# ath92/splat-renderer

Hardware: AMD Instinct MI355X
Metric: Msplats/sec (higher is better)
Workload: dtype f32

## Files before the change

include/splat.h:

```cpp
#ifndef SPLAT_H
#define SPLAT_H

#include <stddef.h>
#include <stdint.h>

#ifdef __cplusplus
extern "C" {
#endif

#define SPLAT_ABI_VERSION 3

#define SPLAT_OK 0
#define SPLAT_ERR_INVALID (-1)
#define SPLAT_ERR_HIP (-2)
#define SPLAT_ERR_OOM (-3)
#define SPLAT_ERR_CAPACITY (-4)
#define SPLAT_ERR_STATE (-5)
#define SPLAT_ERR_NO_DEVICE (-6)
#define SPLAT_ERR_COMM (-7)
#define SPLAT_ERR_RETRY (-8)

typedef struct splat_ctx splat_ctx;
typedef struct splat_sorter splat_sorter;
typedef struct splat_binner splat_binner;
typedef struct splat_comm splat_comm;

#define SPLAT_PROPS_BYTES 32
#define SPLAT_PROJECTED_BYTES 32
#define SPLAT_SORT_BLOCK 3840

enum {
    SPLAT_STAGE_PROJECT = 0,
    SPLAT_STAGE_SORT = 1,
    SPLAT_STAGE_BIN = 2,
    SPLAT_STAGE_COMPOSITE = 3,
    SPLAT_STAGE_EXCHANGE = 4,
    SPLAT_STAGE_BIN_SCATTER = 5,
    SPLAT_STAGE_BIN_PASS2 = 6,
    SPLAT_STAGE_BIN_TILE_SORT = 7,
    SPLAT_STAGE_COUNT = 8
};

int splat_ctx_create(int device_ordinal, splat_ctx **out);
int splat_ctx_create_on_stream(int device_ordinal, void *hip_stream, splat_ctx **out);
void splat_ctx_destroy(splat_ctx *ctx);
const char *splat_last_error(splat_ctx *ctx);
int splat_sync(splat_ctx *ctx);
int splat_abi_version(void);
int splat_set_timing(splat_ctx *ctx, int enabled);
#define SPLAT_TIMING_COUNT_ENTRIES 0x80000000u
int splat_set_timing_stages(splat_ctx *ctx, uint32_t stage_mask);
int splat_set_timing_sampling(splat_ctx *ctx, uint32_t every);
int splat_stage_time_ms(splat_ctx *ctx, int stage, float *ms);
int splat_stage_time_stats(splat_ctx *ctx, int stage, uint32_t *samples, double *total_ms);
int splat_timing_consumed(splat_ctx *ctx, uint64_t *staged, uint64_t *consumed);

int splat_buf_alloc(splat_ctx *ctx, size_t bytes, void **dptr);
int splat_buf_free(splat_ctx *ctx, void *dptr);
int splat_buf_upload(splat_ctx *ctx, void *dst_dptr, const void *src_host, size_t bytes);
int splat_buf_download(splat_ctx *ctx, void *dst_host, const void *src_dptr, size_t bytes);
int splat_buf_zero(splat_ctx *ctx, void *dptr, size_t bytes);
int splat_buf_copy(splat_ctx *ctx, void *dst_dptr, const void *src_dptr, size_t bytes);

int splat_update_props(splat_ctx *ctx, const void *positions, const void *curvature, uint32_t n,
                       void *props);
int splat_update_props_planes(splat_ctx *ctx, const void *positions, const void *curvature, uint32_t n,
                              void *pos_radius, void *color_opacity);
int splat_props_to_planes(splat_ctx *ctx, const void *props, uint32_t n, void *pos_radius, void *color_opacity);

int splat_project(splat_ctx *ctx, const float *uniforms, const void *pos_radius,
                  uint32_t pr_stride_vec4, uint32_t n, void *projected, void *keys, void *payload,
                  uint32_t n_padded);

int splat_extract_keys(splat_ctx *ctx, const void *projected, uint32_t n, uint32_t n_padded,
                       void *keys, void *payload);

int splat_sort_create(splat_ctx *ctx, uint32_t capacity, splat_sorter **out);
void splat_sort_destroy(splat_sorter *s);
uint32_t splat_sort_capacity(const splat_sorter *s);
void *splat_sort_keys(splat_sorter *s);
void *splat_sort_payload(splat_sorter *s);
int splat_sort_run(splat_sorter *s, uint32_t n, uint32_t bit_begin, uint32_t bit_end);
void *splat_sort_sorted_payload(splat_sorter *s);
void *splat_sort_sorted_keys(splat_sorter *s);
int splat_probe_lds_atomic_order(splat_ctx *ctx, uint64_t *mismatches);
int splat_sort_set_mode(splat_sorter *s, int mode);
int splat_rank_status(splat_ctx *ctx, int *policy, int *atomics_ordered, uint32_t *order_faults);
#ifdef SPLAT_TEST_HOOKS
int splat_debug_inject_order_fault(splat_ctx *ctx, uint32_t tile, uint32_t position);
int splat_debug_set_tile_order(splat_ctx *ctx, const void *order_dptr);
int splat_debug_set_tile_sort_order(splat_ctx *ctx, const void *order_dptr);
int splat_debug_rerun_tile_sort(splat_ctx *ctx, splat_binner *binner);
int splat_debug_tile_sort_launches(splat_ctx *ctx, uint32_t *launches);
int splat_debug_lds_rate(splat_ctx *ctx, int kind, uint32_t workgroups_per_cu, uint32_t iters, float *ms);
#endif
int splat_composite_forget_history(splat_ctx *ctx);
int splat_composite_options(splat_ctx *ctx, int kernel, int ahead, int predict);

int splat_scan_u32(splat_ctx *ctx, const void *in, void *out, uint32_t n, void *total_dptr);

int splat_bin_create(splat_ctx *ctx, uint32_t tile_size, splat_binner **out);
void splat_bin_destroy(splat_binner *b);
int splat_bin_run(splat_binner *b, const void *projected, uint32_t n_splats, const void *sorted,
                  uint32_t n_sorted, uint32_t width, uint32_t height, uint32_t tile_row0,
                  uint32_t tile_row1);
uint32_t splat_bin_tile_size(const splat_binner *b);
int splat_bin_counts(splat_binner *b, void **dptr);
int splat_bin_offsets(splat_binner *b, void **dptr);
int splat_bin_indices(splat_binner *b, void **dptr);
int splat_bin_total(splat_binner *b, uint64_t *total_pairs);
#define SPLAT_FRAME_ORDER_DEFAULT (-1)
#define SPLAT_FRAME_SORT_FIRST 0
#define SPLAT_FRAME_TILE_FIRST 1
int splat_bin_set_frame_order(splat_binner *b, int order);
int splat_bin_dims(splat_binner *b, uint32_t *ntx, uint32_t *nty);

int splat_validate_tile_order(splat_ctx *ctx, const void *projected, const void *tile_offsets,
                              uint32_t num_tiles, const void *tile_indices, uint64_t total_pairs,
                              uint64_t *violations_host);

#define SPLAT_COMPOSITE_FRONT_TO_BACK 0
#define SPLAT_COMPOSITE_REFERENCE_LITERAL 1
#define SPLAT_RECORDS_PROJECTED 0
#define SPLAT_RECORDS_COMPACT 1
#define SPLAT_RECORDS_DISC48 2
#define SPLAT_RECORDS_LIT32 3
#define SPLAT_FOOTPRINT_ISOTROPIC 0
#define SPLAT_FOOTPRINT_DISC 1
#define SPLAT_FOOTPRINT_ELLIPSOID 2
#define SPLAT_FOOTPRINT_SURFEL 3
typedef struct splat_composite_cfg {
    uint32_t mode;
    uint32_t early_out;
    uint32_t tile_size;
    uint32_t tile_row0;
    uint32_t tile_row1;
    uint32_t record_format;
    uint32_t prelit;
    uint32_t footprint;
} splat_composite_cfg;
int splat_lit_colors(splat_ctx *ctx, const void *color_opacity, uint32_t color_stride_vec4,
                     const void *normals, uint32_t normal_stride_vec4, uint32_t n, void *lit);
int splat_composite(splat_ctx *ctx, const splat_composite_cfg *cfg, const void *color_opacity,
                    uint32_t color_stride_vec4, const void *normals, uint32_t normal_stride_vec4,
                    const void *projected, const void *tile_indices, const void *tile_counts,
                    const void *tile_offsets, uint32_t width, uint32_t height, void *out_rgba8,
                    void *out_rgba32f, void *consumed_dptr);

typedef struct splat_aov {
    void *depth_f32;
    void *alpha_f32;
    void *id_u32;
} splat_aov;
int splat_composite_aov(splat_ctx *ctx, const splat_composite_cfg *cfg, const void *color_opacity,
                        uint32_t color_stride_vec4, const void *normals, uint32_t normal_stride_vec4,
                        const void *projected, const void *tile_indices, const void *tile_counts,
                        const void *tile_offsets, uint32_t width, uint32_t height, void *out_rgba8,
                        void *out_rgba32f, void *consumed_dptr, const splat_aov *aov);
int splat_composite_aov_depth(splat_ctx *ctx, const splat_composite_cfg *cfg, const void *color_opacity,
                              uint32_t color_stride_vec4, const void *normals, uint32_t normal_stride_vec4,
                              const void *projected, const void *tile_indices, const void *tile_counts,
                              const void *tile_offsets, uint32_t width, uint32_t height, void *out_rgba8,
                              void *out_rgba32f, void *consumed_dptr, const splat_aov *aov, const void *depth_f32,
                              uint32_t depth_stride_floats);

int splat_render_frame(splat_ctx *ctx, splat_sorter *sorter, splat_binner *binner,
                       const splat_composite_cfg *cfg, const float *uniforms, const void *props,
                       const void *normals, uint32_t n, uint32_t width, uint32_t height,
                       void *projected, void *out_rgba8, void *out_rgba32f);
int splat_render_frame_planes(splat_ctx *ctx, splat_sorter *sorter, splat_binner *binner,
                              const splat_composite_cfg *cfg, const float *uniforms,
                              const void *pos_radius, const void *color_opacity, const void *normals,
                              uint32_t n, uint32_t width, uint32_t height, void *projected,
                              void *out_rgba8, void *out_rgba32f);
int splat_render_frame_aov(splat_ctx *ctx, splat_sorter *sorter, splat_binner *binner,
                           const splat_composite_cfg *cfg, const float *uniforms, const void *props,
// ... 257 lines not shown
```

splat_renderer_amd/_lib.py:

```python
import ctypes as C
import os

_HERE = os.path.dirname(os.path.abspath(__file__))
LIB_PATH = os.environ.get("SPLAT_LIB_PATH") or os.path.join(_HERE, "libsplat_hip.so")

OK = 0
ERR_NAMES = {-1: "INVALID", -2: "HIP", -3: "OOM", -4: "CAPACITY", -5: "STATE", -6: "NO_DEVICE", -7: "COMM", -8: "RETRY"}
ERR_CAPACITY, ERR_RETRY = -4, -8
RENDER_AGAIN = (ERR_CAPACITY, ERR_RETRY)

STAGE_PROJECT, STAGE_SORT, STAGE_BIN, STAGE_COMPOSITE, STAGE_EXCHANGE, STAGE_BIN_SCATTER, STAGE_BIN_PASS2, STAGE_BIN_TILE_SORT = range(8)
STAGE_NAMES = ("project", "sort", "bin", "composite", "exchange", "bin_scatter", "bin_second_pass", "bin_tile_sort")
TIMING_COUNT_ENTRIES = 0x80000000
MODE_FRONT_TO_BACK, MODE_REFERENCE_LITERAL = 0, 1
RECORDS_PROJECTED, RECORDS_COMPACT, RECORDS_DISC48, RECORDS_LIT32 = 0, 1, 2, 3
FOOTPRINT_ISOTROPIC, FOOTPRINT_DISC, FOOTPRINT_ELLIPSOID, FOOTPRINT_SURFEL = 0, 1, 2, 3
U32_MAX = 0xFFFFFFFF
DEPTH_DISTANCE, DEPTH_Z = 0, 1


class SplatError(RuntimeError):
    def __init__(self, code, msg):
        super().__init__(f"libsplat_hip error {ERR_NAMES.get(code, code)}: {msg}")
        self.code = code
# ... 117 lines not shown
    "splat_tsdf_mesh_emit": (_i, [_vp, C.POINTER(TsdfGrid), _vp, _vp, _vp, C.c_uint64, _vp, _vp, _vp]),
    "splat_adam_step": (_i, [_vp, _vp, _vp, _vp, _vp, _u32, _u32, _u32, _f64, _f64, _f64, _f64, _f64, _f64, _vp]),
    "splat_density_accumulate": (_i, [_vp, _vp, _vp, _u32, _u32, _u32, _vp, _vp, _vp, _vp]),
    "splat_density_accumulate_abs": (_i, [_vp, _vp, _vp, _u32, _u32, _u32, _vp, _vp, _vp, _vp]),
    "splat_densify_plan_workspace_bytes": (C.c_uint64, [_u32]),
    "splat_densify_plan": (_i, [_vp, _vp, _vp, _vp, _vp, _vp, _u32, C.POINTER(DensifyCfg), _vp, C.c_uint64, _vp, C.POINTER(_u32),
                                C.POINTER(_u32)]),
    "splat_densify_geometry": (_i, [_vp, _vp, _u32, _vp, _vp, _vp, C.POINTER(DensifyCfg), _vp, _vp]),
    "splat_densify_rows": (_i, [_vp, _vp, _u32, _vp, _vp, _u32, _u32]),
    "splat_mcmc_sample_workspace_bytes": (C.c_uint64, [_u32]),
    "splat_mcmc_sample": (_i, [_vp, _vp, _u32, _u32, _u32, _f64, C.c_uint64, _vp, C.c_uint64, _vp, _vp, _vp, C.POINTER(_u32)]),
    "splat_mcmc_apply": (_i, [_vp, _vp, _vp, _vp, _u32, _u32, _u32, _f64, C.POINTER(McmcPlanes)]),
    "splat_mcmc_noise": (_i, [_vp, _vp, _vp, _vp, _vp, _u32, _f64, _u32, C.c_uint64]),
    "splat_knn_workspace_bytes": (C.c_uint64, [_u32]),
    "splat_knn_mean_sq": (_i, [_vp, _vp, _vp, _u32, _u32, _vp, C.c_uint64, _vp, _vp]),
    "splat_extract_keys":(_i, [_vp, _vp, _u32, _u32, _vp, _vp]),
    "splat_sort_create": (_i, [_vp, _u32, _pvp]),
    "splat_sort_destroy": (None, [_vp]),
    "splat_sort_capacity": (_u32, [_vp]),
    "splat_sort_keys": (_vp, [_vp]),
    "splat_sort_payload": (_vp, [_vp]),
    "splat_sort_run": (_i, [_vp, _u32, _u32, _u32]),
    "splat_sort_sorted_payload": (_vp, [_vp]),
    "splat_sort_sorted_keys": (_vp, [_vp]),
    "splat_probe_lds_atomic_order": (_i, [_vp, C.POINTER(C.c_uint64)]),
    "splat_sort_set_mode": (_i, [_vp, _i]),
    "splat_rank_status": (_i, [_vp, C.POINTER(_i), C.POINTER(_i), C.POINTER(_u32)]),
    "splat_composite_forget_history": (_i, [_vp]),
    "splat_composite_options": (_i, [_vp, _i, _i, _i]),
    "splat_scan_u32": (_i, [_vp, _vp, _vp, _u32, _vp]),
    "splat_bin_create": (_i, [_vp, _u32, _pvp]),
    "splat_bin_destroy": (None, [_vp]),
    "splat_bin_run": (_i, [_vp, _vp, _u32, _vp, _u32, _u32, _u32, _u32, _u32]),
    "splat_bin_tile_size": (_u32, [_vp]),
    "splat_bin_counts": (_i, [_vp, _pvp]),
    "splat_bin_offsets": (_i, [_vp, _pvp]),
    "splat_bin_indices": (_i, [_vp, _pvp]),
    "splat_bin_total": (_i, [_vp, C.POINTER(C.c_uint64)]),
    "splat_bin_set_frame_order": (_i, [_vp, _i]),
    "splat_bin_dims": (_i, [_vp, C.POINTER(_u32), C.POINTER(_u32)]),
    "splat_validate_tile_order": (_i, [_vp, _vp, _vp, _u32, _vp, C.c_uint64, C.POINTER(C.c_uint64)]),
    "splat_lit_colors": (_i, [_vp, _vp, _u32, _vp, _u32, _u32, _vp]),
    "splat_composite": (_i, [_vp, C.POINTER(CompositeCfg), _vp, _u32, _vp, _u32, _vp, _vp, _vp, _vp, _u32, _u32,
                             _vp, _vp, _vp]),
    "splat_render_frame": (_i, [_vp, _vp, _vp, C.POINTER(CompositeCfg), C.POINTER(C.c_float), _vp, _vp, _u32, _u32,
                                _u32, _vp, _vp, _vp]),
    "splat_render_frame_planes": (_i, [_vp, _vp, _vp, C.POINTER(CompositeCfg), C.POINTER(C.c_float), _vp, _vp, _vp, _u32,
                                       _u32, _u32, _vp, _vp, _vp]),
    "splat_composite_aov": (_i, [_vp, C.POINTER(CompositeCfg), _vp, _u32, _vp, _u32, _vp, _vp, _vp, _vp, _u32, _u32,
                                 _vp, _vp, _vp, C.POINTER(Aov)]),
    "splat_render_frame_aov": (_i, [_vp, _vp, _vp, C.POINTER(CompositeCfg), C.POINTER(C.c_float), _vp, _vp, _u32, _u32,
                                    _u32, _vp, _vp, _vp, C.POINTER(Aov)]),
    "splat_render_frame_planes_aov": (_i, [_vp, _vp, _vp, C.POINTER(CompositeCfg), C.POINTER(C.c_float), _vp, _vp, _vp,
                                           _u32, _u32, _u32, _vp, _vp, _vp, C.POINTER(Aov)]),
    "splat_project_slice": (_i, [_vp, C.POINTER(C.c_float), _vp, _u32, _u32, _u32, _vp]),
    "splat_project_slice_compact": (_i, [_vp, C.POINTER(C.c_float), _vp, _u32, _u32, _u32, _vp]),
    "splat_project_slice_disc": (_i, [_vp, C.POINTER(C.c_float), _vp, _u32, _vp, _u32, _u32, _u32, _vp]),
    "splat_expand_compact": (_i, [_vp, _vp, _u32, _u32, _vp]),
    "splat_band_frame": (_i, [_vp, _vp, _vp, C.POINTER(CompositeCfg), _vp, _vp, _vp, _u32, _u32, _u32, _vp, _vp, _vp]),
    "splat_band_settle": (_i, [_vp, _vp, _vp, C.POINTER(_u32), C.POINTER(C.c_uint64)]),
    "splat_band_kept": (_i, [_vp, _vp, C.POINTER(_u32)]),
    "splat_band_keys": (_i, [_vp, _vp, _vp, _u32, _u32, _u32, _u32, _u32, _u32, C.POINTER(_u32)]),
    "splat_sdf_gradients": (_i, [_vp, _vp, _u32, _vp, _u32, _vp]),
    "splat_sdf_update_positions": (_i, [_vp, _vp, _vp, _u32, _vp]),
    "splat_sdf_scale_factors": (_i, [_vp, _vp, _u32, _vp, _u32, _vp]),
    "splat_sdf_curvature": (_i, [_vp, _vp, _vp, _u32, _vp]),
    "splat_sdf_seed_positions": (_i, [_vp, C.POINTER(C.c_float), C.POINTER(C.c_float), _u32, C.c_uint64, _vp]),
    "splat_sdf_generate": (_i, [_vp, _vp, _u32, C.POINTER(C.c_float), C.POINTER(C.c_float), C.c_uint64, _vp, _u32, _u32, _vp, _vp, _vp, _vp]),
    "splat_point_frame": (_i, [_vp, _vp, C.POINTER(C.c_float), _vp, _u32, _vp, _u32, _vp, _u32, _u32, _u32, _u32, _vp, _vp, _vp, _vp]),
    "splat_comm_unique_id": (_i, [_vp]),
    "splat_comm_init": (_i, [_vp, _i, _i, _vp, _pvp]),
    "splat_comm_destroy": (None, [_vp]),
    "splat_comm_rank": (_i, [_vp, C.POINTER(_i), C.POINTER(_i)]),
    "splat_comm_count": (_i, [_vp, C.POINTER(_i), C.POINTER(_i)]),
    "splat_allgather_records": (_i, [_vp, _vp, _vp, _vp, _sz]),
}
COMM_ID_BYTES = 128
HOOK_SIGNATURES = {
    "splat_debug_inject_order_fault": (_i, [_vp, _u32, _u32]),
    "splat_debug_set_tile_order": (_i, [_vp, _vp]),
    "splat_debug_set_tile_sort_order": (_i, [_vp, _vp]),
    "splat_debug_rerun_tile_sort": (_i, [_vp, _vp]),
    "splat_debug_tile_sort_launches": (_i, [_vp, C.POINTER(_u32)]),
    "splat_debug_lds_rate": (_i, [_vp, _i, _u32, _u32, C.POINTER(C.c_float)]),
}
HOOKS_LIB_PATH = os.path.join(_HERE, "libsplat_hip_hooks.so")

_lib = None


class _Bound:

    def __getattr__(self, name):
        if name in HOOK_SIGNATURES:
            raise AttributeError(f"libsplat_hip: {name} is a test hook: the shipped library does not carry it; run with "
                                 f"SPLAT_LIB_PATH={HOOKS_LIB_PATH} (the -DSPLAT_TEST_HOOKS build)")
        raise AttributeError(f"libsplat_hip: {name} is not declared in splat_renderer_amd._lib.SIGNATURES")


def load():
    global _lib
    if _lib is not None:
        return _lib
    if not os.path.exists(LIB_PATH):
        raise ImportError(
            f"{LIB_PATH} not found: build it with `python -c 'import __graft_entry__ as g; g.build()'` "
            "(hipcc --offload-arch=gfx950). splat_renderer_amd has no CPU fallback.")
    dll = C.CDLL(LIB_PATH)
    lib = _Bound()
    for name, (res, args) in SIGNATURES.items():
        fn = getattr(dll, name)
        fn.restype = res
        fn.argtypes = args
        setattr(lib, name, fn)
    lib.has_hooks = hasattr(dll, "splat_debug_inject_order_fault")
    if lib.has_hooks:
        for name, (res, args) in HOOK_SIGNATURES.items():
            fn = getattr(dll, name)
            fn.restype = res
            fn.argtypes = args
            setattr(lib, name, fn)
    lib._dll = dll
    _lib = lib
    return lib


def check(rc, ctx=None):
    if rc != OK:
        msg = load().splat_last_error(ctx)
        raise SplatError(rc, msg.decode("utf-8", "replace") if msg else "")
    return rc
```

splat_renderer_amd/csrc/tile_sort.hip:

```cpp
#include "common.h"
#include "block_scan.h"
#include "variant.h"

#include <cstdlib>

constexpr uint32_t TS_THREADS = 256, TS_WAVES = 4;
constexpr uint32_t TS_LONG_ITEMS = 24;
constexpr uint32_t TS_LDS_ELEMS = 5888;
constexpr uint32_t TS_CHUNK_ITEMS = 16;

struct TileSortShared {
    uint32_t wave_hist[TS_WAVES][256];
    uint32_t digit_base[256];
    uint32_t wave_sums[TS_WAVES];
    uint32_t kmin, kmax;
};

__device__ __forceinline__ void tile_list_out(uint2 *s_el, uint32_t n, uint32_t *__restrict__ out, uint32_t *frame_flags, bool inject,
                                              uint32_t inject_pos, uint32_t tid) {
    const uint32_t lane = tid & 63, w = tid >> 6;
    if (inject) {
        if (tid == 0 && n >= inject_pos + 2u) {
            const uint2 a = s_el[inject_pos];
            s_el[inject_pos] = s_el[inject_pos + 1];
            s_el[inject_pos + 1] = a;
        }
        __syncthreads();
    }
    bool bad = false;
    for (uint32_t s0 = 0; s0 * 63u < n; s0 += 4 * TS_WAVES) {
        uint2 a[4];
#pragma unroll
        for (uint32_t i = 0; i < 4; ++i) {
            const uint32_t p = (s0 + i * TS_WAVES + w) * 63u + lane;
            a[i] = s_el[p < n ? p : n - 1];
        }
#pragma unroll
        for (uint32_t i = 0; i < 4; ++i) {
            const uint32_t p = (s0 + i * TS_WAVES + w) * 63u + lane;
            if (p < n && lane < 63) out[p] = a[i].y;
            const uint32_t bx = (uint32_t)__builtin_amdgcn_update_dpp(0, (int)a[i].x, 0x130, 0xf, 0xf, false);
            const uint32_t by = (uint32_t)__builtin_amdgcn_update_dpp(0, (int)a[i].y, 0x130, 0xf, 0xf, false);
#ifndef TS_NO_ORDER_CHECK
            const unsigned long long ka = ((unsigned long long)a[i].x << 32) | a[i].y, kb = ((unsigned long long)bx << 32) | by;
            if (p + 1 < n && lane < 63) bad |= ka >= kb;
#endif
        }
    }
    if (__any(bad) && lane == 0) atomicOr(frame_flags, FRAME_FLAG_ORDER);
}

#ifdef SPLAT_TEST_HOOKS
#define TS_HOOK_PARAMS , uint32_t inject_tile, uint32_t inject_pos, const uint32_t *__restrict__ order
#define TS_HOOK_ARGS , inject, inject_pos, ctx->debug_sort_order
#else
#define TS_HOOK_PARAMS
#define TS_HOOK_ARGS
#endif
template <bool RANK_ATOMIC, uint32_t TS_MAX_ITEMS, bool LAST_CLASS>
__global__ __launch_bounds__(TS_THREADS, TS_MAX_ITEMS <= 8 ? 6 : TS_MAX_ITEMS <= 12 ? 5 : TS_MAX_ITEMS <= 16 ? 4 : 3) void k_tile_sort(const uint32_t *__restrict__ offsets, uint32_t tiles,
                                                                                    uint32_t n_above, uint2 *vals, uint2 *scratch,
                                                                                    uint32_t *__restrict__ out_idx,
                                                                                    uint32_t *__restrict__ counts,
                                                                                    uint32_t *__restrict__ frame_flags TS_HOOK_PARAMS) {
    static_assert(TS_MAX_ITEMS % 4 == 0, "items are processed in groups of four");
    constexpr uint32_t TS_CAP = TS_MAX_ITEMS * TS_THREADS < TS_LDS_ELEMS ? TS_MAX_ITEMS * TS_THREADS : TS_LDS_ELEMS;
    __shared__ TileSortShared sh;
    __shared__ uint2 s_el[TS_CAP];
    uint32_t *run_base = reinterpret_cast<uint32_t *>(s_el);
    const uint32_t tid = threadIdx.x, lane = tid & 63, w = tid >> 6;
#ifdef SPLAT_TEST_HOOKS
    const uint32_t t = order ? order[blockIdx.x] : blockIdx.x;
#else
    const uint32_t t = blockIdx.x;
    constexpr uint32_t inject_tile = 0xffffffffu, inject_pos = 0;
#endif
    const uint32_t base = offsets[t], n = offsets[t + 1] - base;
    if (counts && tid == 0) {
        counts[t] = n;
        if (n > TS_MAX_ITEMS * TS_THREADS) atomicAdd(frame_flags + 2, 1u);
    }
    if (n <= n_above || (!LAST_CLASS && n > TS_CAP)) return;
    uint2 *src = vals + base, *dst = scratch + base;
    const bool in_lds = !LAST_CLASS || n <= TS_CAP;

    if (tid == 0) {
        sh.kmin = 0xffffffffu;
        sh.kmax = 0;
    }
    __syncthreads();

    uint32_t lo = 0xffffffffu, hi = 0;
    const uint32_t items = ((n + TS_THREADS - 1) / TS_THREADS + 3u) & ~3u;
    const uint32_t wbase = w * items * 64 + lane;
    uint2 el[TS_MAX_ITEMS];
    if (in_lds) {
#pragma unroll
        for (uint32_t g = 0; g < TS_MAX_ITEMS; g += 4) {
            if (g < items) {
#pragma unroll
                for (uint32_t i = g; i < g + 4; ++i) {
                    const uint32_t p = wbase + i * 64;
                    el[i] = src[p < n ? p : n - 1];
                }
            }
        }
#pragma unroll
        for (uint32_t g = 0; g < TS_MAX_ITEMS; g += 4) {
            if (g < items) {
#pragma unroll
                for (uint32_t i = g; i < g + 4; ++i) {
                    lo = min(lo, el[i].x);
                    hi = max(hi, el[i].x);
                }
            }
        }
    } else {
        for (uint32_t p = tid; p < n; p += TS_THREADS) {
            const uint32_t k = src[p].x;
            lo = min(lo, k);
            hi = max(hi, k);
        }
    }
#pragma unroll
    for (int d = 32; d >= 1; d >>= 1) {
        lo = min(lo, (uint32_t)__shfl_xor((int)lo, d));
        hi = max(hi, (uint32_t)__shfl_xor((int)hi, d));
    }
    if (lane == 0) {
        atomicMin(&sh.kmin, lo);
        atomicMax(&sh.kmax, hi);
    }
    __syncthreads();
    const uint32_t kmin = sh.kmin, range = sh.kmax - kmin;
    const uint32_t passes = range == 0 ? 0u : (32u - (uint32_t)__builtin_clz(range) + 7u) / 8u;

    if (in_lds) {
        if (passes == 0) {
#pragma unroll
            for (uint32_t g = 0; g < TS_MAX_ITEMS; g += 4) {
                if (g < items) {
#pragma unroll
                    for (uint32_t i = g; i < g + 4; ++i)
                        if (wbase + i * 64 < n) s_el[wbase + i * 64] = el[i];
                }
            }
            __syncthreads();
        }
        for (uint32_t pass = 0; pass < passes; ++pass) {
            const uint32_t shift = pass * 8;
            for (uint32_t i = tid; i < TS_WAVES * 256; i += TS_THREADS) (&sh.wave_hist[0][0])[i] = 0;
            __syncthreads();
            uint32_t rank[TS_MAX_ITEMS];
#pragma unroll
            for (uint32_t g = 0; g < TS_MAX_ITEMS; g += 4) {
                if (g < items) {
                    if (pass > 0) {
#pragma unroll
                        for (uint32_t i = g; i < g + 4; ++i) {
                            const uint32_t p = wbase + i * 64;
                            el[i] = s_el[p < n ? p : n - 1];
                        }
                    }
#pragma unroll
                    for (uint32_t i = g; i < g + 4; ++i) {
                        const uint32_t p = wbase + i * 64;
                        rank[i] = 0;
                        if (p < n) rank[i] = wave_rank<RANK_ATOMIC>(sh.wave_hist[w], ((el[i].x - kmin) >> shift) & 255u);
                    }
                }
            }
            __syncthreads();
            const uint32_t c0 = sh.wave_hist[0][tid], c1 = sh.wave_hist[1][tid], c2 = sh.wave_hist[2][tid], c3 = sh.wave_hist[3][tid];
            const uint32_t excl = block_exclusive_scan<true>((c0 + c1) + (c2 + c3), sh.wave_sums);
            sh.wave_hist[0][tid] = excl;
            sh.wave_hist[1][tid] = excl + c0;
            sh.wave_hist[2][tid] = excl + c0 + c1;
            sh.wave_hist[3][tid] = excl + c0 + c1 + c2;
            __syncthreads();
#pragma unroll
            for (uint32_t g = 0; g < TS_MAX_ITEMS; g += 4) {
                if (g < items) {
                    uint32_t pos[4];
#pragma unroll
                    for (uint32_t i = g; i < g + 4; ++i) pos[i - g] = sh.wave_hist[w][((el[i].x - kmin) >> shift) & 255u] + rank[i];
#pragma unroll
                    for (uint32_t i = g; i < g + 4; ++i)
                        if (wbase + i * 64 < n) s_el[pos[i - g]] = el[i];
                }
            }
            __syncthreads();
        }
        tile_list_out(s_el, n, out_idx + base, frame_flags, t == inject_tile, inject_pos, tid);
        return;
    }

    constexpr uint32_t CH_ITEMS = TS_MAX_ITEMS < TS_CHUNK_ITEMS ? TS_MAX_ITEMS : TS_CHUNK_ITEMS;
    for (uint32_t pass = 0; pass < passes; ++pass) {
        const uint32_t shift = pass * 8;
        sh.digit_base[tid] = 0;
        __syncthreads();
        for (uint32_t p = tid; p < n; p += TS_THREADS) atomicAdd(&sh.digit_base[((src[p].x - kmin) >> shift) & 255u], 1u);
        __syncthreads();
        const uint32_t tot = sh.digit_base[tid];
        const uint32_t start = block_exclusive_scan<true>(tot, sh.wave_sums);
        run_base[tid] = start;
        __syncthreads();
        for (uint32_t c0 = 0; c0 < n; c0 += CH_ITEMS * TS_THREADS) {
            for (uint32_t i = tid; i < TS_WAVES * 256; i += TS_THREADS) (&sh.wave_hist[0][0])[i] = 0;
            __syncthreads();
            uint2 el[CH_ITEMS];
            uint32_t rank[CH_ITEMS];
#pragma unroll
            for (uint32_t i = 0; i < CH_ITEMS; ++i) {
                const uint32_t p = c0 + w * (CH_ITEMS * 64) + i * 64 + lane;
                el[i] = src[p < n ? p : n - 1];
                rank[i] = 0;
                if (p < n) rank[i] = wave_rank<RANK_ATOMIC>(sh.wave_hist[w], ((el[i].x - kmin) >> shift) & 255u);
            }
            __syncthreads();
            const uint32_t dcount = ts_wave_prefixes(sh.wave_hist, tid);
            const uint32_t rb = run_base[tid];
            sh.digit_base[tid] = rb;
            run_base[tid] = rb + dcount;
            __syncthreads();
#pragma unroll
            for (uint32_t i = 0; i < CH_ITEMS; ++i) {
                const uint32_t p = c0 + w * (CH_ITEMS * 64) + i * 64 + lane;
                if (p < n) {
                    const uint32_t d = ((el[i].x - kmin) >> shift) & 255u;
                    dst[sh.digit_base[d] + sh.wave_hist[w][d] + rank[i]] = el[i];
                }
            }
            __syncthreads();
        }
        uint2 *tmp = src; src = dst; dst = tmp;
        __threadfence_block();
        __syncthreads();
    }
    bool bad = false;
    for (uint32_t p = tid; p < n; p += TS_THREADS) {
        const bool inj = t == inject_tile && n >= inject_pos + 2u;
        uint2 a = src[p];
        if (inj && (p == inject_pos || p == inject_pos + 1)) a = src[p == inject_pos ? p + 1 : p - 1];
        out_idx[base + p] = a.y;
        if (p + 1 < n) {
            uint2 b = src[p + 1];
            if (inj && (p + 1 == inject_pos || p + 1 == inject_pos + 1)) b = src[p + 1 == inject_pos ? p + 2 : p];
            bad |= a.x > b.x || (a.x == b.x && a.y >= b.y);
        }
    }
    if (__any(bad) && lane == 0) atomicOr(frame_flags, FRAME_FLAG_ORDER);
}

int tile_sort_launch(splat_ctx *ctx, const TileSortArgs &a) {
    uint32_t *const counts = a.counts, *const short_class_io = a.short_class_io;
    {
        int prc = ctx_resolve_rank_mode(ctx);
        if (prc != SPLAT_OK) return prc;
    }
    const bool ra = rank_atomic_ok(ctx, true);
#ifdef SPLAT_TEST_HOOKS
    const uint32_t inject = ctx->inject_order_fault ? ctx->inject_order_fault - 1u : 0xffffffffu;
    const uint32_t inject_pos = ctx->inject_order_position;
    ctx->inject_order_fault = 0;
#endif
    const bool one_class = (a.band_tiles ? a.band_tiles : a.tiles) <= 4200u;
    static const uint32_t force_short = [] {
        const char *e = getenv("SPLAT_TILE_SORT_SHORT");
        const int v = e ? atoi(e) : 0;
        return (v == 8 || v == 12 || v == 16) ? (uint32_t)v : 0u;
    }();
    const uint32_t short_items = force_short ? force_short : a.mean_list < 320u ? 8u : a.mean_list < 1152u ? 12u : 16u;
    const uint32_t short_cap = short_items * TS_THREADS;
    auto launch_class = [&](uint32_t items, bool last, uint32_t above, uint32_t *class_counts) {
        return variant_dispatch(
            [&](auto ra_, auto items_, auto last_) {
                if constexpr (items_.value != (int)TS_LONG_ITEMS || last_.value) {
                    launch_kernel(ctx, NO_STAGE, k_tile_sort<ra_.value, (uint32_t)items_.value, last_.value>, dim3(a.tiles), dim3(TS_THREADS), a.offsets,
                                  a.tiles, above, a.vals, a.scratch, a.out_idx, class_counts, a.frame_flags TS_HOOK_ARGS);
                    return true;
                } else return false;
            },
            ra, OneOf<8, 12, 16, (int)TS_LONG_ITEMS>{(int)items}, last);
    };
    bool ok, no_long = false;
    if (one_class) {
        ok = launch_class(TS_LONG_ITEMS, true, 0u, counts);
    } else {
        no_long = a.long_tiles_hint == 0u && short_class_io && *short_class_io == short_items;
        if (short_class_io) *short_class_io = short_items;
        ok = launch_class(short_items, no_long, 0u, counts);
        if (ok && !no_long) ok = launch_class(TS_LONG_ITEMS, true, short_cap, nullptr);
    }
    if (!ok) return ctx_fail(ctx, SPLAT_ERR_INVALID, "k_tile_sort: no kernel for this class");
#ifdef SPLAT_TEST_HOOKS
    ctx->tile_sort_launches = one_class || no_long ? 1u : 2u;
#endif
    LAUNCH_CHECK(ctx, "k_tile_sort");
    return SPLAT_OK;
}

#ifdef SPLAT_TEST_HOOKS
extern "C" int splat_debug_set_tile_sort_order(splat_ctx *ctx, const void *order_dptr) {
    if (!ctx) return ctx_fail(nullptr, SPLAT_ERR_INVALID, "ctx is NULL");
    ctx->debug_sort_order = (const uint32_t *)order_dptr;
    return SPLAT_OK;
}

extern "C" int splat_debug_tile_sort_launches(splat_ctx *ctx, uint32_t *launches) {
    if (!ctx || !launches) return ctx_fail(nullptr, SPLAT_ERR_INVALID, "ctx/launches is NULL");
    *launches = ctx->tile_sort_launches;
    return SPLAT_OK;
}

extern "C" int splat_debug_inject_order_fault(splat_ctx *ctx, uint32_t tile, uint32_t position) {
    if (!ctx) return ctx_fail(nullptr, SPLAT_ERR_INVALID, "ctx is NULL");
    ARG_CHECK(ctx, tile != 0xffffffffu);
    ARG_CHECK(ctx, position < 0x3fffffffu);
    ctx->inject_order_fault = tile + 1u;
    ctx->inject_order_position = position;
    return SPLAT_OK;
}
#endif
```

splat_renderer_amd/host.py:

```python
import ctypes as C

import numpy as np

from . import _lib
from ._lib import CompositeCfg, SplatError, check

U32_MAX = 0xFFFFFFFF


class Buffer:

    def __init__(self, device, ptr, size, owned=True):
        self.device, self.ptr, self.size, self._owned = device, ptr, int(size), owned
        self._host_shadow = None

    def destroy(self):
        if self._owned and self.ptr:
            check(self.device.lib.splat_buf_free(self.device.ctx, self.ptr), self.device.ctx)
        self.ptr = None

    def write(self, array, offset=0):
        a = np.ascontiguousarray(array)
        if offset + a.nbytes > self.size:
            raise ValueError("write past the end of the buffer")
# ... 19 lines not shown


class _Queue:
    def __init__(self, device):
        self._d = device

    def writeBuffer(self, buffer, offset, data):
        buffer.write(data, offset)

    def submit(self, _command_buffers=None):
        pass

    def onSubmittedWorkDone(self):
        self._d.sync()


class CommandEncoder:

    def finish(self):
        return None


class Device:

    def __init__(self, ordinal=0, stream=None):
        self.lib = _lib.load()
        p = C.c_void_p()
        if stream is None:
            check(self.lib.splat_ctx_create(ordinal, C.byref(p)))
        else:
            check(self.lib.splat_ctx_create_on_stream(ordinal, C.c_void_p(stream), C.byref(p)))
        self.ctx = p
        self.ordinal = ordinal
        self.queue = _Queue(self)
        self.lastProjector = None
        self.lastBinner = None

    def createBuffer(self, size):
        p = C.c_void_p()
        check(self.lib.splat_buf_alloc(self.ctx, int(size), C.byref(p)), self.ctx)
        return Buffer(self, p.value, size)

    def createBufferFrom(self, array):
        a = np.ascontiguousarray(array)
        return self.createBuffer(max(a.nbytes, 16)).write(a)

    def wrap(self, ptr, size):
        return Buffer(self, int(ptr), size, owned=False)

    def createCommandEncoder(self):
        return CommandEncoder()

    def sync(self):
        check(self.lib.splat_sync(self.ctx), self.ctx)

    def setTiming(self, enabled=True):
        check(self.lib.splat_set_timing(self.ctx, int(enabled)), self.ctx)

    def stageTimeMs(self, stage):
        ms = C.c_float()
        check(self.lib.splat_stage_time_ms(self.ctx, stage, C.byref(ms)), self.ctx)
        return float(ms.value)

    def rankStatus(self):
        pol, ordered, faults = C.c_int(), C.c_int(), C.c_uint32()
        check(self.lib.splat_rank_status(self.ctx, C.byref(pol), C.byref(ordered), C.byref(faults)), self.ctx)
        return {"policy": ("checked", "atomic", "ballot")[pol.value], "atomicsOrdered": bool(ordered.value == 1),
                "orderFaults": int(faults.value)}

    def forgetCompositeHistory(self):
        check(self.lib.splat_composite_forget_history(self.ctx), self.ctx)

    def compositeOptions(self, kernel=None, ahead=0, predict=None):
        k = -1 if kernel is None else {"quadrant": 0, "pixel": 1}[kernel]
        check(self.lib.splat_composite_options(self.ctx, k, int(ahead), -1 if predict is None else int(bool(predict))), self.ctx)

    def injectOrderFault(self, tile, position=0):
        check(self.lib.splat_debug_inject_order_fault(self.ctx, int(tile), int(position)), self.ctx)

    def tileSortLaunches(self):
        v = C.c_uint32(0)
        check(self.lib.splat_debug_tile_sort_launches(self.ctx, C.byref(v)), self.ctx)
        return int(v.value)

    def destroy(self):
        if self.ctx:
            self.lib.splat_ctx_destroy(self.ctx)
            self.ctx = None


def _uniform_floats(u):
    if isinstance(u, Buffer):
        if u._host_shadow is None:
            raise SplatError(-1, "uniform buffer was never written")
        u = u._host_shadow.view(np.float32)
    u = np.ascontiguousarray(u, dtype=np.float32)
    return u


class PointManager:

    def __init__(self, device, scene, seed=0, seeding="device"):
        self.device = device
        self.scene, self._seed, self._positions = None, seed, None
        if seeding not in ("device", "host"):
            raise SplatError(-1, f"seeding must be 'device' or 'host', not {seeding!r}")
        self.seeding = seeding
        if hasattr(scene, "getPrimitives"):
            from . import sdf
            if not scene.getPrimitives():
                raise SplatError(-1, "Scene must have at least one primitive")
            self.scene = scene
            self.numPoints = sdf.point_count(scene)
        else:
            if isinstance(scene, (int, np.integer)):
                from .scene import make_scene
                props, _ = make_scene(int(scene))
                scene = np.concatenate([props[:, :3], np.ones((props.shape[0], 1), np.float32)], axis=1)
            self._positions = np.ascontiguousarray(scene, dtype=np.float32)
            self.numPoints = self._positions.shape[0]
        self._buffers = [device.createBuffer(self.numPoints * 16), device.createBuffer(self.numPoints * 16)]
        self._current = 0
        self.reinitialize()

    def reinitialize(self):
        if self.scene is not None:
            from . import sdf
            if self.seeding == "device":
                mn, mx = sdf.seeding_box(self.scene)
                fp = C.POINTER(C.c_float)
                check(self.device.lib.splat_sdf_seed_positions(self.device.ctx, mn.ctypes.data_as(fp), mx.ctypes.data_as(fp), self.numPoints,
                                                               int(self._seed) & 0xFFFFFFFFFFFFFFFF, self._buffers[self._current].ptr),
                      self.device.ctx)
                self._seed += 1
                return
            self._positions = sdf.seed_positions(self.scene, self.numPoints, self._seed)
            self._seed += 1
        self._buffers[self._current].write(self._positions)

    def swap(self):
        self._current = 1 - self._current

    def getCurrentPositionBuffer(self):
        return self._buffers[self._current]

    def getNextPositionBuffer(self):
        return self._buffers[1 - self._current]

    def getNumPoints(self):
        return self.numPoints

    def destroy(self):
        for b in self._buffers:
            b.destroy()


class PropertyPlanes:

    def __init__(self, posRadius, colorOpacity, prelit=False, ownsPosRadius=True):
        self.posRadius, self.colorOpacity, self.prelit, self._owns_pos = posRadius, colorOpacity, prelit, ownsPosRadius

    def destroy(self):
        if self._owns_pos:
            self.posRadius.destroy()
        self.colorOpacity.destroy()

# ... 804 lines not shown
```

Baseline: 15650.

## Alias tile-sort shared state into element LDS and pack ranks to raise occupancy

The tile-sort kernel now overlays its histogram and scan scratch onto the element array in LDS instead of allocating both, and raises the launch-bounds occupancy target for each item class. Ranks are packed two per register in 16-bit halves, keys are pre-offset by kmin, and the per-wave key min/max is gathered through slots instead of LDS atomics. A DPP-based wave scan replaces the generic block scan. The global-memory fallback is split into its own function, and a debug hook reports occupancy. Aliasing forces extra barriers, and the tighter register budget may cause spills.

```diff
diff --git a/include/splat.h b/include/splat.h
--- a/include/splat.h
+++ b/include/splat.h
@@ -92,6 +92,7 @@
 int splat_debug_set_tile_sort_order(splat_ctx *ctx, const void *order_dptr);
 int splat_debug_rerun_tile_sort(splat_ctx *ctx, splat_binner *binner);
 int splat_debug_tile_sort_launches(splat_ctx *ctx, uint32_t *launches);
+int splat_debug_tile_sort_occupancy(splat_ctx *ctx, uint32_t items, int last, int ballot, uint32_t *workgroups_per_cu, uint32_t *lds_cap);
 int splat_debug_lds_rate(splat_ctx *ctx, int kind, uint32_t workgroups_per_cu, uint32_t iters, float *ms);
 #endif
 int splat_composite_forget_history(splat_ctx *ctx);
diff --git a/splat_renderer_amd/_lib.py b/splat_renderer_amd/_lib.py
--- a/splat_renderer_amd/_lib.py
+++ b/splat_renderer_amd/_lib.py
@@ -223,6 +223,7 @@
     "splat_debug_set_tile_sort_order": (_i, [_vp, _vp]),
     "splat_debug_rerun_tile_sort": (_i, [_vp, _vp]),
     "splat_debug_tile_sort_launches": (_i, [_vp, C.POINTER(_u32)]),
+    "splat_debug_tile_sort_occupancy": (_i, [_vp, _u32, _i, _i, C.POINTER(_u32), C.POINTER(_u32)]),
     "splat_debug_lds_rate": (_i, [_vp, _i, _u32, _u32, C.POINTER(C.c_float)]),
 }
 HOOKS_LIB_PATH = os.path.join(_HERE, "libsplat_hip_hooks.so")
diff --git a/splat_renderer_amd/csrc/tile_sort.hip b/splat_renderer_amd/csrc/tile_sort.hip
--- a/splat_renderer_amd/csrc/tile_sort.hip
+++ b/splat_renderer_amd/csrc/tile_sort.hip
@@ -8,13 +8,48 @@
 constexpr uint32_t TS_LONG_ITEMS = 24;
 constexpr uint32_t TS_LDS_ELEMS = 5888;
 constexpr uint32_t TS_CHUNK_ITEMS = 16;
+constexpr uint32_t ts_class_cap(uint32_t items) { return items * TS_THREADS < TS_LDS_ELEMS ? items * TS_THREADS : TS_LDS_ELEMS; }
+constexpr uint32_t ts_class_workgroups(uint32_t items) { return items <= 8 ? 8 : items <= 12 ? 6 : items <= 16 ? 5 : 3; }
 
 struct TileSortShared {
     uint32_t wave_hist[TS_WAVES][256];
     uint32_t digit_base[256];
+    uint32_t run_base[256];
     uint32_t wave_sums[TS_WAVES];
-    uint32_t kmin, kmax;
+    uint32_t kmin_w[TS_WAVES], kmax_w[TS_WAVES];
 };
+static_assert(sizeof(TileSortShared) <= 8 * TS_THREADS * sizeof(uint2), "the view must fit the smallest class's element array (8 per thread, 16 KiB)");
+
+__device__ __forceinline__ uint32_t ts_fresh_v(uint32_t v) {
+    asm volatile("" : "+v"(v));
+    return v;
+}
+__device__ __forceinline__ uint32_t ts_fresh_s(uint32_t v) {
+    asm volatile("" : "+s"(v));
+    return v;
+}
+
+template <int CTRL, int ROW_MASK>
+__device__ __forceinline__ uint32_t ts_dpp_add(uint32_t x) {
+    return x + (uint32_t)__builtin_amdgcn_update_dpp(0, (int)x, CTRL, ROW_MASK, 0xf, false);
+}
+__device__ __forceinline__ uint32_t ts_wave_inclusive_scan(uint32_t x) {
+    x = ts_dpp_add<0x111, 0xf>(x);
+    x = ts_dpp_add<0x112, 0xf>(x);
+    x = ts_dpp_add<0x114, 0xf>(x);
+    x = ts_dpp_add<0x118, 0xf>(x);
+    x = ts_dpp_add<0x142, 0xa>(x);
+    x = ts_dpp_add<0x143, 0xc>(x);
+    return x;
+}
+__device__ __forceinline__ uint32_t ts_block_exclusive_scan(uint32_t v, uint32_t *wave_sums, uint32_t lane, uint32_t w) {
+    const uint32_t incl = ts_wave_inclusive_scan(v);
+    if (lane == 63) wave_sums[w] = incl;
+    __syncthreads();
+    const uint32_t before = waves_before(wave_sums, w);
+    __syncthreads();
+    return before + incl - v;
+}
 
 __device__ __forceinline__ void tile_list_out(uint2 *s_el, uint32_t n, uint32_t *__restrict__ out, uint32_t *frame_flags, bool inject,
                                               uint32_t inject_pos, uint32_t tid) {
@@ -50,152 +85,33 @@
     if (__any(bad) && lane == 0) atomicOr(frame_flags, FRAME_FLAG_ORDER);
 }
 
-#ifdef SPLAT_TEST_HOOKS
-#define TS_HOOK_PARAMS , uint32_t inject_tile, uint32_t inject_pos, const uint32_t *__restrict__ order
-#define TS_HOOK_ARGS , inject, inject_pos, ctx->debug_sort_order
-#else
-#define TS_HOOK_PARAMS
-#define TS_HOOK_ARGS
-#endif
-template <bool RANK_ATOMIC, uint32_t TS_MAX_ITEMS, bool LAST_CLASS>
-__global__ __launch_bounds__(TS_THREADS, TS_MAX_ITEMS <= 8 ? 6 : TS_MAX_ITEMS <= 12 ? 5 : TS_MAX_ITEMS <= 16 ? 4 : 3) void k_tile_sort(const uint32_t *__restrict__ offsets, uint32_t tiles,
-                                                                                    uint32_t n_above, uint2 *vals, uint2 *scratch,
-                                                                                    uint32_t *__restrict__ out_idx,
-                                                                                    uint32_t *__restrict__ counts,
-                                                                                    uint32_t *__restrict__ frame_flags TS_HOOK_PARAMS) {
-    static_assert(TS_MAX_ITEMS % 4 == 0, "items are processed in groups of four");
-    constexpr uint32_t TS_CAP = TS_MAX_ITEMS * TS_THREADS < TS_LDS_ELEMS ? TS_MAX_ITEMS * TS_THREADS : TS_LDS_ELEMS;
-    __shared__ TileSortShared sh;
-    __shared__ uint2 s_el[TS_CAP];
-    uint32_t *run_base = reinterpret_cast<uint32_t *>(s_el);
-    const uint32_t tid = threadIdx.x, lane = tid & 63, w = tid >> 6;
-#ifdef SPLAT_TEST_HOOKS
-    const uint32_t t = order ? order[blockIdx.x] : blockIdx.x;
-#else
-    const uint32_t t = blockIdx.x;
-    constexpr uint32_t inject_tile = 0xffffffffu, inject_pos = 0;
-#endif
-    const uint32_t base = offsets[t], n = offsets[t + 1] - base;
-    if (counts && tid == 0) {
-        counts[t] = n;
-        if (n > TS_MAX_ITEMS * TS_THREADS) atomicAdd(frame_flags + 2, 1u);
-    }
-    if (n <= n_above || (!LAST_CLASS && n > TS_CAP)) return;
-    uint2 *src = vals + base, *dst = scratch + base;
-    const bool in_lds = !LAST_CLASS || n <= TS_CAP;
-
-    if (tid == 0) {
-        sh.kmin = 0xffffffffu;
-        sh.kmax = 0;
-    }
-    __syncthreads();
-
-    uint32_t lo = 0xffffffffu, hi = 0;
-    const uint32_t items = ((n + TS_THREADS - 1) / TS_THREADS + 3u) & ~3u;
-    const uint32_t wbase = w * items * 64 + lane;
-    uint2 el[TS_MAX_ITEMS];
-    if (in_lds) {
-#pragma unroll
-        for (uint32_t g = 0; g < TS_MAX_ITEMS; g += 4) {
-            if (g < items) {
-#pragma unroll
-                for (uint32_t i = g; i < g + 4; ++i) {
-                    const uint32_t p = wbase + i * 64;
-                    el[i] = src[p < n ? p : n - 1];
-                }
-            }
-        }
-#pragma unroll
-        for (uint32_t g = 0; g < TS_MAX_ITEMS; g += 4) {
-            if (g < items) {
-#pragma unroll
-                for (uint32_t i = g; i < g + 4; ++i) {
-                    lo = min(lo, el[i].x);
-                    hi = max(hi, el[i].x);
-                }
-            }
-        }
-    } else {
-        for (uint32_t p = tid; p < n; p += TS_THREADS) {
-            const uint32_t k = src[p].x;
-            lo = min(lo, k);
-            hi = max(hi, k);
-        }
-    }
+__device__ __forceinline__ uint32_t ts_key_range(TileSortShared &sh, uint32_t lo, uint32_t hi, uint32_t lane, uint32_t w, uint32_t &kmin) {
 #pragma unroll
     for (int d = 32; d >= 1; d >>= 1) {
         lo = min(lo, (uint32_t)__shfl_xor((int)lo, d));
         hi = max(hi, (uint32_t)__shfl_xor((int)hi, d));
     }
     if (lane == 0) {
-        atomicMin(&sh.kmin, lo);
-        atomicMax(&sh.kmax, hi);
+        sh.kmin_w[w] = lo;
+        sh.kmax_w[w] = hi;
     }
     __syncthreads();
-    const uint32_t kmin = sh.kmin, range = sh.kmax - kmin;
-    const uint32_t passes = range == 0 ? 0u : (32u - (uint32_t)__builtin_clz(range) + 7u) / 8u;
-
-    if (in_lds) {
-        if (passes == 0) {
-#pragma unroll
-            for (uint32_t g = 0; g < TS_MAX_ITEMS; g += 4) {
-                if (g < items) {
-#pragma unroll
-                    for (uint32_t i = g; i < g + 4; ++i)
-                        if (wbase + i * 64 < n) s_el[wbase + i * 64] = el[i];
-                }
-            }
-            __syncthreads();
-        }
-        for (uint32_t pass = 0; pass < passes; ++pass) {
-            const uint32_t shift = pass * 8;
-            for (uint32_t i = tid; i < TS_WAVES * 256; i += TS_THREADS) (&sh.wave_hist[0][0])[i] = 0;
-            __syncthreads();
-            uint32_t rank[TS_MAX_ITEMS];
-#pragma unroll
-            for (uint32_t g = 0; g < TS_MAX_ITEMS; g += 4) {
-                if (g < items) {
-                    if (pass > 0) {
-#pragma unroll
-                        for (uint32_t i = g; i < g + 4; ++i) {
-                            const uint32_t p = wbase + i * 64;
-                            el[i] = s_el[p < n ? p : n - 1];
-                        }
-                    }
-#pragma unroll
-                    for (uint32_t i = g; i < g + 4; ++i) {
-                        const uint32_t p = wbase + i * 64;
-                        rank[i] = 0;
-                        if (p < n) rank[i] = wave_rank<RANK_ATOMIC>(sh.wave_hist[w], ((el[i].x - kmin) >> shift) & 255u);
-                    }
-                }
-            }
-            __syncthreads();
-            const uint32_t c0 = sh.wave_hist[0][tid], c1 = sh.wave_hist[1][tid], c2 = sh.wave_hist[2][tid], c3 = sh.wave_hist[3][tid];
-            const uint32_t excl = block_exclusive_scan<true>((c0 + c1) + (c2 + c3), sh.wave_sums);
-            sh.wave_hist[0][tid] = excl;
-            sh.wave_hist[1][tid] = excl + c0;
-            sh.wave_hist[2][tid] = excl + c0 + c1;
-            sh.wave_hist[3][tid] = excl + c0 + c1 + c2;
-            __syncthreads();
-#pragma unroll
-            for (uint32_t g = 0; g < TS_MAX_ITEMS; g += 4) {
-                if (g < items) {
-                    uint32_t pos[4];
-#pragma unroll
-                    for (uint32_t i = g; i < g + 4; ++i) pos[i - g] = sh.wave_hist[w][((el[i].x - kmin) >> shift) & 255u] + rank[i];
-#pragma unroll
-                    for (uint32_t i = g; i < g + 4; ++i)
-                        if (wbase + i * 64 < n) s_el[pos[i - g]] = el[i];
-                }
-            }
-            __syncthreads();
-        }
-        tile_list_out(s_el, n, out_idx + base, frame_flags, t == inject_tile, inject_pos, tid);
-        return;
-    }
-
-    constexpr uint32_t CH_ITEMS = TS_MAX_ITEMS < TS_CHUNK_ITEMS ? TS_MAX_ITEMS : TS_CHUNK_ITEMS;
+    kmin = min(min(sh.kmin_w[0], sh.kmin_w[1]), min(sh.kmin_w[2], sh.kmin_w[3]));
+    const uint32_t range = max(max(sh.kmax_w[0], sh.kmax_w[1]), max(sh.kmax_w[2], sh.kmax_w[3])) - kmin;
+    return range == 0 ? 0u : (32u - (uint32_t)__builtin_clz(range) + 7u) / 8u;
+}
+
+template <bool RANK_ATOMIC, uint32_t CH_ITEMS>
+__device__ __forceinline__ void tile_sort_through_global(TileSortShared &sh, uint2 *src, uint2 *dst, uint32_t n, uint32_t *__restrict__ out,
+                                                         uint32_t *frame_flags, bool inject, uint32_t inject_pos, uint32_t tid, uint32_t lane,
+                                                         uint32_t w) {
+    uint32_t lo = 0xffffffffu, hi = 0, kmin;
+    for (uint32_t p = tid; p < n; p += TS_THREADS) {
+        const uint32_t k = src[p].x;
+        lo = min(lo, k);
+        hi = max(hi, k);
+    }
+    const uint32_t passes = ts_key_range(sh, lo, hi, lane, w, kmin);
     for (uint32_t pass = 0; pass < passes; ++pass) {
         const uint32_t shift = pass * 8;
         sh.digit_base[tid] = 0;
@@ -203,8 +119,8 @@
         for (uint32_t p = tid; p < n; p += TS_THREADS) atomicAdd(&sh.digit_base[((src[p].x - kmin) >> shift) & 255u], 1u);
         __syncthreads();
         const uint32_t tot = sh.digit_base[tid];
-        const uint32_t start = block_exclusive_scan<true>(tot, sh.wave_sums);
-        run_base[tid] = start;
+        const uint32_t start = ts_block_exclusive_scan(tot, sh.wave_sums, lane, w);
+        sh.run_base[tid] = start;
         __syncthreads();
         for (uint32_t c0 = 0; c0 < n; c0 += CH_ITEMS * TS_THREADS) {
             for (uint32_t i = tid; i < TS_WAVES * 256; i += TS_THREADS) (&sh.wave_hist[0][0])[i] = 0;
@@ -220,9 +136,9 @@
             }
             __syncthreads();
             const uint32_t dcount = ts_wave_prefixes(sh.wave_hist, tid);
-            const uint32_t rb = run_base[tid];
+            const uint32_t rb = sh.run_base[tid];
             sh.digit_base[tid] = rb;
-            run_base[tid] = rb + dcount;
+            sh.run_base[tid] = rb + dcount;
             __syncthreads();
 #pragma unroll
             for (uint32_t i = 0; i < CH_ITEMS; ++i) {
@@ -240,10 +156,10 @@
     }
     bool bad = false;
     for (uint32_t p = tid; p < n; p += TS_THREADS) {
-        const bool inj = t == inject_tile && n >= inject_pos + 2u;
+        const bool inj = inject && n >= inject_pos + 2u;
         uint2 a = src[p];
         if (inj && (p == inject_pos || p == inject_pos + 1)) a = src[p == inject_pos ? p + 1 : p - 1];
-        out_idx[base + p] = a.y;
+        out[p] = a.y;
         if (p + 1 < n) {
             uint2 b = src[p + 1];
             if (inj && (p + 1 == inject_pos || p + 1 == inject_pos + 1)) b = src[p + 1 == inject_pos ? p + 2 : p];
@@ -251,6 +167,162 @@
         }
     }
     if (__any(bad) && lane == 0) atomicOr(frame_flags, FRAME_FLAG_ORDER);
+}
+
+#ifdef SPLAT_TEST_HOOKS
+#define TS_HOOK_PARAMS , uint32_t inject_tile, uint32_t inject_pos, const uint32_t *__restrict__ order
+#define TS_HOOK_ARGS , inject, inject_pos, ctx->debug_sort_order
+#else
+#define TS_HOOK_PARAMS
+#define TS_HOOK_ARGS
+#endif
+template <bool RANK_ATOMIC, uint32_t TS_MAX_ITEMS, bool LAST_CLASS>
+__global__ __launch_bounds__(TS_THREADS, ts_class_workgroups(TS_MAX_ITEMS)) void k_tile_sort(const uint32_t *__restrict__ offsets, uint32_t tiles,
+                                                                                    uint32_t n_above, uint2 *vals, uint2 *scratch,
+                                                                                    uint32_t *__restrict__ out_idx,
+                                                                                    uint32_t *__restrict__ counts,
+                                                                                    uint32_t *__restrict__ frame_flags TS_HOOK_PARAMS) {
+    static_assert(TS_MAX_ITEMS % 4 == 0, "items are processed in groups of four");
+    constexpr uint32_t TS_CAP = ts_class_cap(TS_MAX_ITEMS);
+    __shared__ uint2 s_el[TS_CAP];
+    TileSortShared &sh = *reinterpret_cast<TileSortShared *>(s_el);
+    const uint32_t tid = threadIdx.x, lane = tid & 63;
+    const uint32_t w = (uint32_t)__builtin_amdgcn_readfirstlane((int)(tid >> 6));
+#ifdef SPLAT_TEST_HOOKS
+    const uint32_t t = order ? order[blockIdx.x] : blockIdx.x;
+#else
+    const uint32_t t = blockIdx.x;
+    constexpr uint32_t inject_tile = 0xffffffffu, inject_pos = 0;
+#endif
+    const uint32_t base = offsets[t], n = offsets[t + 1] - base;
+    if (counts && tid == 0) {
+        counts[t] = n;
+        if (n > (TS_MAX_ITEMS == TS_LONG_ITEMS ? TS_MAX_ITEMS * TS_THREADS : TS_CAP)) atomicAdd(frame_flags + 2, 1u);
+    }
+    if (n <= n_above || (!LAST_CLASS && n > TS_CAP)) return;
+    uint2 *src = vals + base;
+    if constexpr (LAST_CLASS) {
+        if (n > TS_CAP) {
+            tile_sort_through_global<RANK_ATOMIC, (TS_MAX_ITEMS < TS_CHUNK_ITEMS ? TS_MAX_ITEMS : TS_CHUNK_ITEMS)>(
+                sh, src, scratch + base, n, out_idx + base, frame_flags, t == inject_tile, inject_pos, tid, lane, w);
+            return;
+        }
+    }
+
+    uint32_t lo = 0xffffffffu, hi = 0;
+    const uint32_t items = ((n + TS_THREADS - 1) / TS_THREADS + 3u) & ~3u;
+    const uint32_t wbase = w * items * 64 + lane;
+    uint2 el[TS_MAX_ITEMS];
+#pragma unroll
+    for (uint32_t g = 0; g < TS_MAX_ITEMS; g += 4) {
+        if (g < items) {
+#pragma unroll
+            for (uint32_t i = g; i < g + 4; ++i) {
+                const uint32_t p = wbase + i * 64;
+                el[i] = src[p < n ? p : n - 1];
+            }
+        }
+    }
+#pragma unroll
+    for (uint32_t g = 0; g < TS_MAX_ITEMS; g += 4) {
+        if (g < items) {
+#pragma unroll
+            for (uint32_t i = g; i < g + 4; ++i) {
+                lo = min(lo, el[i].x);
+                hi = max(hi, el[i].x);
+            }
+        }
+    }
+    uint32_t kmin;
+    const uint32_t passes = ts_key_range(sh, lo, hi, lane, w, kmin);
+
+    {
+#pragma unroll
+        for (uint32_t i = 0; i < TS_MAX_ITEMS; ++i) el[i].x -= kmin;
+        if (passes == 0) {
+            __syncthreads();
+#pragma unroll
+            for (uint32_t g = 0; g < TS_MAX_ITEMS; g += 4) {
+                if (g < items) {
+#pragma unroll
+                    for (uint32_t i = g; i < g + 4; ++i)
+                        if (wbase + i * 64 < n) s_el[wbase + i * 64] = el[i];
+                }
+            }
+            __syncthreads();
+        }
+#pragma clang loop unroll(disable)
+        for (uint32_t pass = 0; pass < passes; ++pass) {
+            if (pass > 0) {
+                const uint32_t wb = ts_fresh_v(wbase);
+#pragma unroll
+                for (uint32_t g = 0; g < TS_MAX_ITEMS; g += 4) {
+                    if (g < items) {
+#pragma unroll
+                        for (uint32_t i = g; i < g + 4; ++i) {
+                            const uint32_t p = wb + i * 64;
+                            el[i] = s_el[p < n ? p : n - 1];
+                        }
+                    }
+                }
+                __syncthreads();
+            }
+#pragma unroll
+            for (uint32_t i = 0; i < 4; ++i) sh.wave_hist[w][i * 64 + lane] = 0;
+            uint32_t rank[TS_MAX_ITEMS / 2];
+            {
+                const uint32_t wb = ts_fresh_v(wbase), shift = ts_fresh_s(pass * 8);
+#pragma unroll
+                for (uint32_t g = 0; g < TS_MAX_ITEMS; g += 4) {
+                    if (g < items) {
+                        uint32_t r[4];
+#pragma unroll
+                        for (uint32_t i = g; i < g + 4; ++i) {
+                            r[i - g] = 0;
+                            if (wb + i * 64 < n) r[i - g] = wave_rank<RANK_ATOMIC>(sh.wave_hist[w], (el[i].x >> shift) & 255u);
+                        }
+                        rank[g / 2] = r[0] | (r[1] << 16);
+                        rank[g / 2 + 1] = r[2] | (r[3] << 16);
+                    }
+                }
+            }
+            __syncthreads();
+            const uint32_t c0 = sh.wave_hist[0][tid], c1 = sh.wave_hist[1][tid], c2 = sh.wave_hist[2][tid], c3 = sh.wave_hist[3][tid];
+            const uint32_t excl = ts_block_exclusive_scan((c0 + c1) + (c2 + c3), sh.wave_sums, lane, w);
+            sh.wave_hist[0][tid] = excl;
+            sh.wave_hist[1][tid] = excl + c0;
+            sh.wave_hist[2][tid] = excl + c0 + c1;
+            sh.wave_hist[3][tid] = excl + c0 + c1 + c2;
+            __syncthreads();
+            {
+                const uint32_t shift = ts_fresh_s(pass * 8);
+#pragma unroll
+                for (uint32_t g = 0; g < TS_MAX_ITEMS; g += 4) {
+                    if (g < items) {
+#pragma unroll
+                        for (uint32_t i = g; i < g + 4; i += 2) {
+                            const uint32_t p0 = sh.wave_hist[w][(el[i].x >> shift) & 255u], p1 = sh.wave_hist[w][(el[i + 1].x >> shift) & 255u];
+                            rank[i / 2] += p0 | (p1 << 16);
+                        }
+                    }
+                }
+            }
+            __syncthreads();
+            {
+                const uint32_t wb = ts_fresh_v(wbase);
+#pragma unroll
+                for (uint32_t g = 0; g < TS_MAX_ITEMS; g += 4) {
+                    if (g < items) {
+#pragma unroll
+                        for (uint32_t i = g; i < g + 4; ++i)
+                            if (wb + i * 64 < n) s_el[(rank[i / 2] >> (i % 2 * 16)) & 0xffffu] = el[i];
+                    }
+                }
+            }
+            __syncthreads();
+        }
+        tile_list_out(s_el, n, out_idx + base, frame_flags, t == inject_tile, inject_pos, tid);
+    }
 }
 
 int tile_sort_launch(splat_ctx *ctx, const TileSortArgs &a) {
@@ -272,7 +344,7 @@
         return (v == 8 || v == 12 || v == 16) ? (uint32_t)v : 0u;
     }();
     const uint32_t short_items = force_short ? force_short : a.mean_list < 320u ? 8u : a.mean_list < 1152u ? 12u : 16u;
-    const uint32_t short_cap = short_items * TS_THREADS;
+    const uint32_t short_cap = ts_class_cap(short_items);
     auto launch_class = [&](uint32_t items, bool last, uint32_t above, uint32_t *class_counts) {
         return variant_dispatch(
             [&](auto ra_, auto items_, auto last_) {
@@ -314,6 +386,25 @@
     return SPLAT_OK;
 }
 
+extern "C" int splat_debug_tile_sort_occupancy(splat_ctx *ctx, uint32_t items, int last, int ballot, uint32_t *workgroups_per_cu, uint32_t *lds_cap) {
+    if (!ctx || !workgroups_per_cu || !lds_cap) return ctx_fail(nullptr, SPLAT_ERR_INVALID, "ctx/workgroups_per_cu/lds_cap is NULL");
+    int wg = 0;
+    hipError_t e = hipSuccess;
+    const bool ok = variant_dispatch(
+        [&](auto ra_, auto items_, auto last_) {
+            if constexpr (items_.value != (int)TS_LONG_ITEMS || last_.value) {
+                e = hipOccupancyMaxActiveBlocksPerMultiprocessor(&wg, k_tile_sort<ra_.value, (uint32_t)items_.value, last_.value>, (int)TS_THREADS, 0);
+                return true;
+            } else return false;
+        },
+        ballot == 0, OneOf<8, 12, 16, (int)TS_LONG_ITEMS>{(int)items}, last != 0);
+    if (!ok) return ctx_fail(ctx, SPLAT_ERR_INVALID, "k_tile_sort: no kernel for this class");
+    if (e != hipSuccess) return ctx_fail(ctx, SPLAT_ERR_HIP, "hipOccupancyMaxActiveBlocksPerMultiprocessor", e);
+    *workgroups_per_cu = (uint32_t)wg;
+    *lds_cap = ts_class_cap(items);
+    return SPLAT_OK;
+}
+
 extern "C" int splat_debug_inject_order_fault(splat_ctx *ctx, uint32_t tile, uint32_t position) {
     if (!ctx) return ctx_fail(nullptr, SPLAT_ERR_INVALID, "ctx is NULL");
     ARG_CHECK(ctx, tile != 0xffffffffu);
diff --git a/splat_renderer_amd/host.py b/splat_renderer_amd/host.py
--- a/splat_renderer_amd/host.py
+++ b/splat_renderer_amd/host.py
@@ -125,6 +125,11 @@
         v = C.c_uint32(0)
         check(self.lib.splat_debug_tile_sort_launches(self.ctx, C.byref(v)), self.ctx)
         return int(v.value)
+
+    def tileSortOccupancy(self, items, last, ballot=False):
+        wg, cap = C.c_uint32(0), C.c_uint32(0)
+        check(self.lib.splat_debug_tile_sort_occupancy(self.ctx, int(items), int(bool(last)), int(bool(ballot)), C.byref(wg), C.byref(cap)), self.ctx)
+        return int(wg.value), int(cap.value)
 
     def destroy(self):
         if self.ctx:
```

Result: faster. 15810, median of 6 (+1.0%).
